# guzba/zippy

Hardware: NVIDIA H100
Metric: compress_level1_gzip_input_throughput (higher is better)
Workload: dtype u8

## Files before the change

### include/zippy_b200.h

```cpp
#ifndef ZIPPY_B200_H
#define ZIPPY_B200_H

#include <stddef.h>
#include <stdint.h>

#ifdef __cplusplus
extern "C" {
#endif

enum {
  ZB200_OK = 0,
  ZB200_ERR_INVALID_LEVEL = 1,
  ZB200_ERR_INVALID_FORMAT = 2,
  ZB200_ERR_UNCOMPRESS = 3,
  ZB200_ERR_COMPRESS = 4,
  ZB200_ERR_END_OF_BUFFER = 5,
  ZB200_ERR_BYTE_BOUNDARY = 6,
  ZB200_ERR_BLOCK_HEADER = 7,
  ZB200_ERR_INVALID_SYMBOL = 8,
  ZB200_ERR_DETECT = 9,
  ZB200_ERR_METHOD = 10,
  ZB200_ERR_CINFO = 11,
  ZB200_ERR_HEADER = 12,
  ZB200_ERR_FDICT = 13,
// ... 53 lines not shown
                                int data_format, const uint8_t *dict, size_t dict_len, uint64_t *sizes, int *statuses);
int zb200_uncompress_batch_dict(zb200_ctx *ctx, const uint8_t *src_base, const uint64_t *src_offsets, size_t n,
                                int data_format, const uint8_t *dict, size_t dict_len, uint8_t *dst_base,
                                const uint64_t *dst_offsets, uint64_t *dst_lens, int *statuses);
int zb200_decode_begin_dict(zb200_ctx *ctx, const uint8_t *src, size_t len, int data_format, const uint8_t *dict,
                            size_t dict_len, size_t *out_len);

int zb200_checksum_batch(zb200_ctx *ctx, const uint8_t *src_base, const uint64_t *src_offsets, size_t n,
                         int kind, uint32_t *out);

enum { ZB200_SYNC_FLUSH = 2, ZB200_FULL_FLUSH = 3 };
typedef struct zb200_compress_stream zb200_compress_stream;
int zb200_compress_stream_begin(zb200_ctx *ctx, int level, int data_format, int fname_len, zb200_compress_stream **out);
int zb200_compress_stream_begin_dict(zb200_ctx *ctx, int level, int data_format, const uint8_t *dict, size_t dict_len,
                                     zb200_compress_stream **out);
size_t zb200_compress_stream_bound(const zb200_compress_stream *st, size_t len);
int zb200_compress_stream_write(zb200_compress_stream *st, const uint8_t *src, size_t len,
                                uint8_t *dst, size_t dst_cap, size_t *dst_len);
int zb200_compress_stream_flush(zb200_compress_stream *st, int mode, uint8_t *dst, size_t dst_cap, size_t *dst_len);
int zb200_compress_stream_finish(zb200_compress_stream *st, uint8_t *dst, size_t dst_cap, size_t *dst_len);
void zb200_compress_stream_free(zb200_compress_stream *st);

typedef struct zb200_decompress_stream zb200_decompress_stream;
int zb200_decompress_stream_begin(zb200_ctx *ctx, int data_format, zb200_decompress_stream **out);
int zb200_decompress_stream_begin_dict(zb200_ctx *ctx, int data_format, const uint8_t *dict, size_t dict_len,
                                       zb200_decompress_stream **out);
int zb200_decompress_stream_write(zb200_decompress_stream *st, const uint8_t *src, size_t len, size_t *avail);
int zb200_decompress_stream_drain(zb200_decompress_stream *st, size_t *avail);
int zb200_decompress_stream_finish(zb200_decompress_stream *st, size_t *avail);
int zb200_decompress_stream_read(zb200_decompress_stream *st, uint8_t *dst, size_t dst_cap, size_t *dst_len);
void zb200_decompress_stream_free(zb200_decompress_stream *st);

typedef struct zb200_index zb200_index;
int zb200_index_build(zb200_ctx *ctx, const uint8_t *src, size_t len, int data_format, uint64_t span, zb200_index **out);
int zb200_index_extract_batch(zb200_ctx *ctx, const zb200_index *idx, const uint8_t *src, size_t len,
                              const uint64_t *offsets, const uint64_t *lens, size_t n, uint8_t *dst,
                              const uint64_t *dst_offsets, int *statuses);
uint64_t zb200_index_size(const zb200_index *idx);
size_t zb200_index_points(const zb200_index *idx, uint64_t *bits, uint64_t *outs, uint32_t *crcs, uint8_t *window,
                          size_t cap);
void zb200_index_free(zb200_index *idx);
int zb200_index_export(zb200_ctx *ctx, const zb200_index *idx, uint8_t *dst, size_t cap, size_t *len);
int zb200_index_import(zb200_ctx *ctx, const uint8_t *src, size_t len, zb200_index **out);

int zb200_compress_batch_device(zb200_ctx *ctx, const uint8_t *d_src, const uint64_t *src_offsets, size_t n,
                                int level, int data_format, const uint8_t *fname_lens,
                                uint8_t *d_dst, size_t dst_cap, uint64_t *dst_offsets, int *statuses);
int zb200_compress_batch_h2d(zb200_ctx *ctx, const uint8_t *src_base, const uint64_t *src_offsets, size_t n,
                             int level, int data_format, const uint8_t *fname_lens,
                             uint8_t *d_dst, size_t dst_cap, uint64_t *dst_offsets, int *statuses);
int zb200_download(zb200_ctx *ctx, const uint8_t *d_src, uint8_t *h_dst, size_t bytes);
int zb200_uncompress_batch_device(zb200_ctx *ctx, const uint8_t *d_src, const uint64_t *src_offsets, size_t n,
                                  int data_format, uint8_t *d_dst, const uint64_t *dst_offsets,
                                  uint64_t *dst_lens, int *statuses);
int zb200_uncompress_sizes_device(zb200_ctx *ctx, const uint8_t *d_src, const uint64_t *src_offsets, size_t n,
                                  int data_format, uint64_t *sizes, int *statuses);
int zb200_checksum_batch_device(zb200_ctx *ctx, const uint8_t *d_src, const uint64_t *src_offsets, size_t n,
                                int kind, uint32_t *out);

int zb200_host_register(void *ptr, size_t bytes);
int zb200_host_unregister(void *ptr);

typedef struct zb200_mgpu zb200_mgpu;
int zb200_mgpu_init(const int *devices, int n_devices, zb200_mgpu **out);
void zb200_mgpu_shutdown(zb200_mgpu *m);
int zb200_mgpu_device_count(zb200_mgpu *m);
int zb200_mgpu_compress_batch(zb200_mgpu *m, const uint8_t *src_base, const uint64_t *src_offsets, size_t n,
                              int level, int data_format, const uint8_t *fname_lens,
                              uint8_t *dst_base, size_t dst_cap, uint64_t *dst_offsets, int *statuses);
int zb200_mgpu_uncompress_batch(zb200_mgpu *m, const uint8_t *src_base, const uint64_t *src_offsets, size_t n,
                                int data_format, uint8_t *dst_base, const uint64_t *dst_offsets,
                                uint64_t *dst_lens, int *statuses);
int zb200_mgpu_checksum_batch(zb200_mgpu *m, const uint8_t *src_base, const uint64_t *src_offsets, size_t n,
                              int kind, uint32_t *out);

typedef struct {
  float lz_ms, huff_ms, scan_ms, pack_ms;
  float inflate_ms, verify_ms;
  float checksum_ms;
  float h2d_ms, d2h_ms;
  uint64_t h2d_bytes, d2h_bytes;
  uint32_t kernel_launches;
  uint32_t n_chunks;
} zb200_timing;
int zb200_last_timing(zb200_ctx *ctx, zb200_timing *out);

#ifdef __cplusplus
}
#endif
#endif
```

### zippy_b200/_native.py

```python
import ctypes
import os

_HERE = os.path.dirname(os.path.abspath(__file__))
LIB_PATH = os.path.join(_HERE, "libzippy_b200.so")

c_u8p = ctypes.c_void_p
c_u64p = ctypes.c_void_p
c_intp = ctypes.c_void_p
c_size_t = ctypes.c_size_t
c_int = ctypes.c_int


class Timing(ctypes.Structure):
    _fields_ = [("lz_ms", ctypes.c_float), ("huff_ms", ctypes.c_float), ("scan_ms", ctypes.c_float),
                ("pack_ms", ctypes.c_float), ("inflate_ms", ctypes.c_float), ("verify_ms", ctypes.c_float),
                ("checksum_ms", ctypes.c_float), ("h2d_ms", ctypes.c_float), ("d2h_ms", ctypes.c_float),
                ("h2d_bytes", ctypes.c_uint64), ("d2h_bytes", ctypes.c_uint64),
                ("kernel_launches", ctypes.c_uint32), ("n_chunks", ctypes.c_uint32)]


SYMBOLS = {
    "zb200_init": (c_int, [c_int, ctypes.POINTER(ctypes.c_void_p)]),
    "zb200_shutdown": (None, [ctypes.c_void_p]),
    "zb200_strerror": (ctypes.c_char_p, [c_int]),
    "zb200_last_cuda_error": (ctypes.c_char_p, [ctypes.c_void_p]),
    "zb200_device_count": (c_int, []),
    "zb200_set_stream": (c_int, [ctypes.c_void_p, ctypes.c_void_p]),
    "zb200_deflate_bound": (c_size_t, [c_size_t]),
    "zb200_compress_bound": (c_size_t, [c_size_t, c_int]),
    "zb200_deflate": (c_int, [ctypes.c_void_p, c_u8p, c_size_t, c_int, c_u8p, c_size_t, ctypes.POINTER(c_size_t)]),
    "zb200_inflate": (c_int, [ctypes.c_void_p, c_u8p, c_size_t, c_size_t, c_u8p, c_size_t, ctypes.POINTER(c_size_t)]),
    "zb200_inflate_size": (c_int, [ctypes.c_void_p, c_u8p, c_size_t, c_size_t, ctypes.POINTER(c_size_t)]),
    "zb200_decode_begin": (c_int, [ctypes.c_void_p, c_u8p, c_size_t, c_int, c_size_t, ctypes.POINTER(c_size_t)]),
    "zb200_decode_finish": (c_int, [ctypes.c_void_p, c_u8p, c_size_t, ctypes.POINTER(c_size_t)]),
    "zb200_crc32": (c_int, [ctypes.c_void_p, c_u8p, c_size_t, ctypes.POINTER(ctypes.c_uint32)]),
    "zb200_adler32": (c_int, [ctypes.c_void_p, c_u8p, c_size_t, ctypes.POINTER(ctypes.c_uint32)]),
    "zb200_compress_batch": (c_int, [ctypes.c_void_p, c_u8p, c_u64p, c_size_t, c_int, c_int, c_u8p, c_u8p, c_size_t,
                                     c_u64p, c_intp]),
    "zb200_compress_batch_h2d": (c_int, [ctypes.c_void_p, c_u8p, c_u64p, c_size_t, c_int, c_int, c_u8p, c_u8p, c_size_t,
                                         c_u64p, c_intp]),
    "zb200_download": (c_int, [ctypes.c_void_p, c_u8p, c_u8p, c_size_t]),
    "zb200_host_register": (c_int, [ctypes.c_void_p, c_size_t]),
    "zb200_host_unregister": (c_int, [ctypes.c_void_p]),
    "zb200_uncompress_sizes": (c_int, [ctypes.c_void_p, c_u8p, c_u64p, c_size_t, c_int, c_u64p, c_intp]),
    "zb200_uncompress_batch": (c_int, [ctypes.c_void_p, c_u8p, c_u64p, c_size_t, c_int, c_u8p, c_u64p, c_u64p, c_intp]),
    "zb200_inflate_batch_crc32": (c_int, [ctypes.c_void_p, c_u8p, c_u64p, c_size_t, c_u8p, c_u64p, c_u64p,
                                          ctypes.c_void_p, c_intp]),
    "zb200_checksum_batch": (c_int, [ctypes.c_void_p, c_u8p, c_u64p, c_size_t, c_int, ctypes.c_void_p]),
    "zb200_compress_batch_dict": (c_int, [ctypes.c_void_p, c_u8p, c_u64p, c_size_t, c_int, c_int, c_u8p, c_size_t, c_u8p,
                                          c_size_t, c_u64p, c_intp]),
    "zb200_uncompress_sizes_dict": (c_int, [ctypes.c_void_p, c_u8p, c_u64p, c_size_t, c_int, c_u8p, c_size_t, c_u64p,
                                            c_intp]),
    "zb200_uncompress_batch_dict": (c_int, [ctypes.c_void_p, c_u8p, c_u64p, c_size_t, c_int, c_u8p, c_size_t, c_u8p,
                                            c_u64p, c_u64p, c_intp]),
    "zb200_decode_begin_dict": (c_int, [ctypes.c_void_p, c_u8p, c_size_t, c_int, c_u8p, c_size_t,
                                        ctypes.POINTER(c_size_t)]),
    "zb200_compress_batch_device": (c_int, [ctypes.c_void_p, c_u8p, c_u64p, c_size_t, c_int, c_int, c_u8p, c_u8p,
                                            c_size_t, c_u64p, c_intp]),
    "zb200_uncompress_batch_device": (c_int, [ctypes.c_void_p, c_u8p, c_u64p, c_size_t, c_int, c_u8p, c_u64p, c_u64p,
                                              c_intp]),
    "zb200_uncompress_sizes_device": (c_int, [ctypes.c_void_p, c_u8p, c_u64p, c_size_t, c_int, c_u64p, c_intp]),
    "zb200_checksum_batch_device": (c_int, [ctypes.c_void_p, c_u8p, c_u64p, c_size_t, c_int, ctypes.c_void_p]),
    "zb200_compress_stream_begin": (c_int, [ctypes.c_void_p, c_int, c_int, c_int, ctypes.POINTER(ctypes.c_void_p)]),
    "zb200_compress_stream_begin_dict": (c_int, [ctypes.c_void_p, c_int, c_int, c_u8p, c_size_t,
                                                 ctypes.POINTER(ctypes.c_void_p)]),
    "zb200_compress_stream_bound": (c_size_t, [ctypes.c_void_p, c_size_t]),
    "zb200_compress_stream_write": (c_int, [ctypes.c_void_p, c_u8p, c_size_t, c_u8p, c_size_t, ctypes.POINTER(c_size_t)]),
    "zb200_compress_stream_flush": (c_int, [ctypes.c_void_p, c_int, c_u8p, c_size_t, ctypes.POINTER(c_size_t)]),
    "zb200_compress_stream_finish": (c_int, [ctypes.c_void_p, c_u8p, c_size_t, ctypes.POINTER(c_size_t)]),
    "zb200_compress_stream_free": (None, [ctypes.c_void_p]),
    "zb200_decompress_stream_begin": (c_int, [ctypes.c_void_p, c_int, ctypes.POINTER(ctypes.c_void_p)]),
    "zb200_decompress_stream_begin_dict": (c_int, [ctypes.c_void_p, c_int, c_u8p, c_size_t,
                                                   ctypes.POINTER(ctypes.c_void_p)]),
    "zb200_decompress_stream_write": (c_int, [ctypes.c_void_p, c_u8p, c_size_t, ctypes.POINTER(c_size_t)]),
    "zb200_decompress_stream_drain": (c_int, [ctypes.c_void_p, ctypes.POINTER(c_size_t)]),
    "zb200_decompress_stream_finish": (c_int, [ctypes.c_void_p, ctypes.POINTER(c_size_t)]),
    "zb200_decompress_stream_read": (c_int, [ctypes.c_void_p, c_u8p, c_size_t, ctypes.POINTER(c_size_t)]),
    "zb200_decompress_stream_free": (None, [ctypes.c_void_p]),
    "zb200_index_build": (c_int, [ctypes.c_void_p, c_u8p, c_size_t, c_int, ctypes.c_uint64,
                                  ctypes.POINTER(ctypes.c_void_p)]),
    "zb200_index_extract_batch": (c_int, [ctypes.c_void_p, ctypes.c_void_p, c_u8p, c_size_t, c_u64p, c_u64p, c_size_t,
                                          c_u8p, c_u64p, c_intp]),
    "zb200_index_size": (ctypes.c_uint64, [ctypes.c_void_p]),
    "zb200_index_points": (c_size_t, [ctypes.c_void_p, c_u64p, c_u64p, ctypes.c_void_p, c_u8p, c_size_t]),
    "zb200_index_free": (None, [ctypes.c_void_p]),
    "zb200_index_export": (c_int, [ctypes.c_void_p, ctypes.c_void_p, c_u8p, c_size_t, ctypes.POINTER(c_size_t)]),
    "zb200_index_import": (c_int, [ctypes.c_void_p, c_u8p, c_size_t, ctypes.POINTER(ctypes.c_void_p)]),
    "zb200_mgpu_init": (c_int, [ctypes.c_void_p, c_int, ctypes.POINTER(ctypes.c_void_p)]),
    "zb200_mgpu_shutdown": (None, [ctypes.c_void_p]),
    "zb200_mgpu_device_count": (c_int, [ctypes.c_void_p]),
    "zb200_mgpu_compress_batch": (c_int, [ctypes.c_void_p, c_u8p, c_u64p, c_size_t, c_int, c_int, c_u8p, c_u8p, c_size_t,
                                          c_u64p, c_intp]),
    "zb200_mgpu_uncompress_batch": (c_int, [ctypes.c_void_p, c_u8p, c_u64p, c_size_t, c_int, c_u8p, c_u64p, c_u64p, c_intp]),
    "zb200_mgpu_checksum_batch": (c_int, [ctypes.c_void_p, c_u8p, c_u64p, c_size_t, c_int, ctypes.c_void_p]),
    "zb200_last_timing": (c_int, [ctypes.c_void_p, ctypes.POINTER(Timing)]),
}

_lib = None


def lib():
# ... 14 lines not shown
```

### zippy_b200/csrc/zb_api.cu

```cuda
#include <cuda.h>
#include <cuda_runtime.h>
#include <execinfo.h>
#include <signal.h>
#include <stdio.h>
#include <unistd.h>
#include <stdlib.h>
#include <string.h>

#include <algorithm>
#include <cmath>
#include <condition_variable>
#include <deque>
#include <functional>
#include <memory>
#include <mutex>
#include <thread>
#include <string>
#include <vector>

#include "../../include/zippy_b200.h"
#include "zb_kernels.h"
#include "zb_wrapper.h"

namespace {

struct DevBuf {
  void *p = nullptr;
  size_t cap = 0;
};

struct StreamMemOps {
  CUresult (*wait32)(CUstream, CUdeviceptr, cuuint32_t, unsigned int) = nullptr;
  CUresult (*write32)(CUstream, CUdeviceptr, cuuint32_t, unsigned int) = nullptr;
  bool ok = false;
};
StreamMemOps load_stream_memops() {
  StreamMemOps m;
  void *f1 = nullptr, *f2 = nullptr;
  cudaDriverEntryPointQueryResult q1, q2;
  if (cudaGetDriverEntryPoint("cuStreamWaitValue32", &f1, cudaEnableDefault, &q1) == cudaSuccess && q1 == cudaDriverEntryPointSuccess &&
      cudaGetDriverEntryPoint("cuStreamWriteValue32", &f2, cudaEnableDefault, &q2) == cudaSuccess && q2 == cudaDriverEntryPointSuccess &&
      f1 && f2) {
    m.wait32 = reinterpret_cast<decltype(m.wait32)>(f1);
    m.write32 = reinterpret_cast<decltype(m.write32)>(f2);
    m.ok = true;
  } else {
    (void)cudaGetLastError();
  }
  return m;
}

constexpr size_t kMaxChunksPerGroup = 32768;
constexpr size_t kHostGroupChunks = 4096;
constexpr size_t ZB_STREAM_BATCH_BYTES = 64u << 20;
constexpr size_t ZB_DSTREAM_BATCH_BYTES = 64u << 20;
constexpr uint64_t kDstreamMaxOut = 1ull << 30;

}

class CopyPool {
 public:
  ~CopyPool() { stop(); }
  void start(int n) {
    if (!th_.empty()) return;
    for (int i = 0; i < n; i++) th_.emplace_back([this] { work(); });
  }
  void stop() {
    {
      std::lock_guard<std::mutex> lk(m_);
      quit_ = true;
    }
    cv_.notify_all();
    for (std::thread &t : th_) t.join();
    th_.clear();
  }
  void copy(uint8_t *dst, const uint8_t *src, size_t n) {
    const size_t piece = 1 << 20;
    if (th_.empty() || n < 2 * piece) {
      memcpy(dst, src, n);
      return;
    }
    {
      std::lock_guard<std::mutex> lk(m_);
      dst_ = dst;
      src_ = src;
      n_ = n;
      next_ = 0;
      left_ = (n + piece - 1) / piece;
    }
    cv_.notify_all();
    help(piece);
    std::unique_lock<std::mutex> lk(m_);
// ... 231 lines not shown
  return a.type == cudaMemoryTypeUnregistered;
}

int ring_ready(zb200_ctx *ctx, StageRing &r) {
  if (r.slot[0]) return ZB200_OK;
  for (int i = 0; i < kStageSlots; i++) {
    if (cudaMallocHost((void **)&r.slot[i], kStageSlotBytes) != cudaSuccess ||
        cudaEventCreateWithFlags(&r.ev[i], cudaEventDisableTiming) != cudaSuccess) {
      cudaGetLastError();
      ctx->last_err = "pinned staging ring: allocation failed";
      return ZB200_ERR_NOMEM;
    }
  }
  unsigned hc = std::thread::hardware_concurrency();
  ctx->pool.start((int)std::min<unsigned>(7, hc > 2 ? hc / 2 : 1));
  return ZB200_OK;
}

int h2d_copy(zb200_ctx *ctx, uint8_t *d_dst, const uint8_t *h_src, size_t n, cudaStream_t st, bool pageable) {
  if (!n) return ZB200_OK;
  if (!pageable) {
    CK(cudaMemcpyAsync(d_dst, h_src, n, cudaMemcpyHostToDevice, st));
    return ZB200_OK;
  }
  StageRing &r = ctx->ring_in;
  int rc = ring_ready(ctx, r);
  if (rc) return rc;
  for (size_t off = 0; off < n; off += kStageSlotBytes) {
    const size_t len = std::min(kStageSlotBytes, n - off);
    const size_t k = r.next++ % kStageSlots;
    if (r.busy[k]) CK(cudaEventSynchronize(r.ev[k]));
    ctx->pool.copy(r.slot[k], h_src + off, len);
    CK(cudaMemcpyAsync(d_dst + off, r.slot[k], len, cudaMemcpyHostToDevice, st));
    CK(cudaEventRecord(r.ev[k], st));
    r.busy[k] = true;
  }
  return ZB200_OK;
}

int d2h_complete(zb200_ctx *ctx, size_t k) {
  StageRing &r = ctx->ring_out;
  if (!r.busy[k]) return ZB200_OK;
  CK(cudaEventSynchronize(r.ev[k]));
  ctx->pool.copy(r.out_dst[k], r.slot[k], r.out_n[k]);
  r.busy[k] = false;
  return ZB200_OK;
}
int d2h_flush(zb200_ctx *ctx) {
  if (!ctx->ring_out.slot[0]) return ZB200_OK;
  for (size_t i = 0; i < (size_t)kStageSlots; i++) {
    int rc = d2h_complete(ctx, (ctx->ring_out.next + i) % kStageSlots);
    if (rc) return rc;
  }
  return ZB200_OK;
}
int d2h_copy(zb200_ctx *ctx, uint8_t *h_dst, const uint8_t *d_src, size_t n, cudaStream_t st, bool pageable) {
  if (!n) return ZB200_OK;
  if (!pageable) {
    CK(cudaMemcpyAsync(h_dst, d_src, n, cudaMemcpyDeviceToHost, st));
    return ZB200_OK;
  }
  StageRing &r = ctx->ring_out;
  int rc = ring_ready(ctx, r);
  if (rc) return rc;
  for (size_t off = 0; off < n; off += kStageSlotBytes) {
    const size_t len = std::min(kStageSlotBytes, n - off);
    const size_t k = r.next++ % kStageSlots;
    rc = d2h_complete(ctx, k);
    if (rc) return rc;
    CK(cudaMemcpyAsync(r.slot[k], d_src + off, len, cudaMemcpyDeviceToHost, st));
    CK(cudaEventRecord(r.ev[k], st));
    r.busy[k] = true;
    r.out_dst[k] = h_dst + off;
    r.out_n[k] = len;
  }
  return ZB200_OK;
}

struct Group {
  size_t m0, m1;
  size_t c0, nc;
  size_t first0;
  uint64_t in_lo, in_hi;
  uint64_t bound;
};

struct StreamPart {
  uint32_t hist;
  bool head, last;
  ZbMemberCarry carry_in, carry_out;
  bool has_dict;
  uint32_t dict_id;
};

uint32_t host_adler32(const uint8_t *p, size_t n) {
  uint64_t a = 1, b = 0;
  while (n) {
    const size_t k = std::min<size_t>(n, 5552);
    for (size_t i = 0; i < k; i++) {
      a += p[i];
      b += a;
    }
    a %= 65521;
    b %= 65521;
    p += k;
    n -= k;
  }
  return (uint32_t)(b << 16 | a);
}

struct DictScope {
  zb200_ctx *ctx;
  explicit DictScope(zb200_ctx *c) : ctx(c) {}
  int set(const uint8_t *dict, size_t dict_len, bool lz_compress = false) {
    if (!dict_len) return ZB200_OK;
    zb200_ctx *ctx = this->ctx;
    const uint32_t wl = (uint32_t)std::min<size_t>(dict_len, 32768);
    const uint8_t *w = dict + (dict_len - wl);
    if (lz_compress) {
      const uint32_t stride = zb_win16_stride(wl);
      std::vector<uint8_t> h16((size_t)16 * stride, 0);
      for (uint32_t c = 0; c < 16; c++) memcpy(h16.data() + (size_t)c * stride + ZB_WIN16_SLACK + ((c - wl) & 15u), w, wl);
      ENSURE(ctx->dict_win16, h16.size() + 64);
      CK(cudaMemcpyAsync(ctx->dict_win16.p, h16.data(), h16.size(), cudaMemcpyHostToDevice, ctx->stream));
      CK(cudaStreamSynchronize(ctx->stream));
    } else {
      ENSURE(ctx->dict_win, wl + 64);
      CK(cudaMemcpyAsync(ctx->dict_win.p, w, wl, cudaMemcpyHostToDevice, ctx->stream));
      CK(cudaStreamSynchronize(ctx->stream));
    }
    ctx->dict_len = wl;
    ctx->dict_id = host_adler32(dict, dict_len);
    ctx->dict_on = true;
    return ZB200_OK;
  }
  ~DictScope() { ctx->dict_on = false; }
};

int compress_locked(zb200_ctx *ctx, const uint8_t *d_src, const uint8_t *h_src, const uint64_t *src_offsets,
                    size_t n, int level, int data_format, const uint8_t *fname_lens, uint8_t *d_dst,
                    size_t dst_cap, uint8_t *h_dst, size_t h_dst_cap, uint64_t *dst_offsets, int *statuses,
                    size_t max_group_chunks, StreamPart *sp = nullptr) {
  if (level < -2 || level > 9) return ZB200_ERR_INVALID_LEVEL;
  if (data_format != ZB200_DF_GZIP && data_format != ZB200_DF_ZLIB && data_format != ZB200_DF_DEFLATE)
    return ZB200_ERR_INVALID_FORMAT;
  if (fname_lens)
    for (size_t i = 0; i < n; i++)
      if (fname_lens[i] > 25) return ZB200_ERR_ARG;
  if (((uintptr_t)d_dst & 3u) != 0) return ZB200_ERR_ARG;
  dst_cap &= ~(size_t)3;
  for (size_t i = 0; i < n; i++) {
    if (src_offsets[i + 1] < src_offsets[i]) return ZB200_ERR_ARG;
    if (statuses) statuses[i] = ZB200_OK;
  }
  ctx->timing.lz_ms = ctx->timing.huff_ms = ctx->timing.scan_ms = ctx->timing.pack_ms = 0.f;
  ctx->timing.n_chunks = 0;
  dst_offsets[0] = 0;
  if (n == 0) return ZB200_OK;
  const uint64_t hist = sp ? sp->hist : 0;
  const bool head = !sp || sp->head, last = !sp || sp->last;
  const bool lz = level == -1 || level >= 2;
  const bool dict_hist = !sp && ctx->dict_on && lz;
  const bool has_dict = data_format == ZB200_DF_ZLIB && (sp ? sp->has_dict : ctx->dict_on);
  const uint32_t dict_id = sp ? sp->dict_id : ctx->dict_id;
  const uint64_t src_lo = src_offsets[0] - hist;
  const bool src_pageable = h_src && is_pageable(h_src + src_lo), dst_pageable = h_dst && is_pageable(h_dst);

  std::vector<Group> groups;
  std::vector<ZbChunkDesc> desc;
  std::vector<uint32_t> first;
  size_t max_nc = 0, max_nm = 0;
  size_t chunks_left = 0;
  for (size_t i = 0; i < n; i++) {
    uint64_t len = src_offsets[i + 1] - src_offsets[i];
    chunks_left += len == 0 ? 1 : (size_t)((len + ZB_CHUNK_BYTES - 1) / ZB_CHUNK_BYTES);
  }
  const size_t group_cap = max_group_chunks;
  for (size_t m0 = 0; m0 < n;) {
    if (h_src) max_group_chunks = std::min(group_cap, std::max<size_t>(512, chunks_left / 2));
    Group g;
    g.m0 = m0;
    g.c0 = desc.size();
    g.first0 = first.size();
    g.bound = 0;
    size_t m1 = m0;
    while (m1 < n) {
      uint64_t len = src_offsets[m1 + 1] - src_offsets[m1];
      size_t nc = len == 0 ? 1 : (size_t)((len + ZB_CHUNK_BYTES - 1) / ZB_CHUNK_BYTES);
      if (desc.size() > g.c0 && desc.size() - g.c0 + nc > max_group_chunks) break;
      first.push_back((uint32_t)(desc.size() - g.c0));
      for (size_t k = 0; k < nc; k++) {
        ZbChunkDesc d;
        d.src_off = src_offsets[m1] - (h_src ? src_lo : 0) + (uint64_t)k * ZB_CHUNK_BYTES;
        d.len = (uint32_t)std::min<uint64_t>(ZB_CHUNK_BYTES, len - (uint64_t)k * ZB_CHUNK_BYTES);
        d.member = (uint32_t)(m1 - m0);
        d.flags = (k == 0 ? ZB_CHUNK_FIRST | (head ? ZB_CHUNK_HEAD : 0u) : 0u) | (k == nc - 1 && last ? ZB_CHUNK_LAST : 0u);
        d.pad = lz ? (uint32_t)std::min<uint64_t>(32768, hist + (uint64_t)k * ZB_CHUNK_BYTES) : 0u;
        if (dict_hist && k == 0) {
          d.pad = ctx->dict_len;
          d.flags |= ZB_CHUNK_DICT;
        }
        desc.push_back(d);
      }
      g.bound += zb200_compress_bound((size_t)len, data_format) + 64;
      m1++;
    }
    g.m1 = m1;
    g.nc = desc.size() - g.c0;
    chunks_left -= std::min(chunks_left, g.nc);
    first.push_back((uint32_t)g.nc);
    g.in_lo = m0 == 0 ? 0 : src_offsets[m0] - src_lo;
    g.in_hi = src_offsets[m1] - src_lo;
    max_nc = std::max(max_nc, g.nc);
    max_nm = std::max(max_nm, g.m1 - g.m0);
    groups.push_back(g);
    m0 = m1;
  }
  const size_t ng = groups.size(), nc_all = desc.size(), nfirst = first.size();

  ENSURE(ctx->desc, nc_all * sizeof(ZbChunkDesc));
  ENSURE(ctx->member_first, nfirst * sizeof(uint32_t));
  ENSURE(ctx->member_off, nfirst * sizeof(uint64_t));
  ENSURE(ctx->fname, n + 16);
  ENSURE(ctx->group_end, (ng + 1) * sizeof(uint64_t));
  ENSURE(ctx->masks, max_nc * ZB_WINDOWS_PER_CHUNK * sizeof(uint2));
  ENSURE(ctx->recs, max_nc * (size_t)ZB_RECS_PER_CHUNK * sizeof(uint32_t));
  ENSURE(ctx->hist, max_nc * (size_t)ZB_WARPS_PER_CHUNK * ZB_HIST_SYMS * sizeof(uint16_t));
  ENSURE(ctx->chk, max_nc * sizeof(ZbChunkCheck));
  ENSURE(ctx->cb, max_nc * sizeof(ZbCodebook));
  ENSURE(ctx->chunk_off, max_nc * sizeof(uint64_t));
  ENSURE(ctx->member_check, max_nm * sizeof(uint32_t));
  ENSURE(ctx->member_isize, max_nm * sizeof(uint32_t));
  if (lz) ENSURE(ctx->lz2_tables, zb_lz2_table_bytes(nullptr));
  if (sp) ENSURE(ctx->carry, 2 * sizeof(ZbMemberCarry));
  {
    int rc = ensure_pinned(ctx, nfirst * sizeof(uint64_t) + sizeof(ZbMemberCarry) + 64);
    if (rc) return rc;
    rc = ensure_group_events(ctx, 3 * ng + 1);
    if (rc) return rc;
  }
  uint64_t *pin_off = (uint64_t *)ctx->pin;
  ZbMemberCarry *pin_carry = (ZbMemberCarry *)(pin_off + nfirst);
  ZbMemberCarry *d_carry = (ZbMemberCarry *)ctx->carry.p;

  cudaStream_t s = ctx->stream;
  cudaStream_t sh = h_src ? ctx->h2d_stream : s, sd = h_dst ? ctx->d2h_stream : s;
  CK(cudaMemcpyAsync(ctx->desc.p, desc.data(), nc_all * sizeof(ZbChunkDesc), cudaMemcpyHostToDevice, s));
  CK(cudaMemcpyAsync(ctx->member_first.p, first.data(), nfirst * sizeof(uint32_t), cudaMemcpyHostToDevice, s));
  if (fname_lens && data_format == ZB200_DF_GZIP)
    CK(cudaMemcpyAsync(ctx->fname.p, fname_lens, n, cudaMemcpyHostToDevice, s));
  if (sp) CK(cudaMemcpyAsync(d_carry, &sp->carry_in, sizeof(ZbMemberCarry), cudaMemcpyHostToDevice, s));
  CK(cudaMemsetAsync(ctx->group_end.p, 0, sizeof(uint64_t), s));
  if (h_src || h_dst) {
    CK(cudaEventRecord(ctx->gev[3 * ng], s));
    if (h_src) CK(cudaStreamWaitEvent(sh, ctx->gev[3 * ng], 0));
    if (h_dst) CK(cudaStreamWaitEvent(sd, ctx->gev[3 * ng], 0));
  }
  CK(cudaEventRecord(ctx->ev[6], sh));

  auto make_work = [&](const Group &g, size_t gi) {
    ZbCompressWork w;
    w.src = d_src;
    w.dst = d_dst;
    w.dst_cap = dst_cap;
    w.desc = (const ZbChunkDesc *)ctx->desc.p + g.c0;
    w.member_first = (const uint32_t *)ctx->member_first.p + g.first0;
    w.fname_len = (fname_lens && data_format == ZB200_DF_GZIP) ? (const uint8_t *)ctx->fname.p + g.m0 : nullptr;
    w.masks = (uint2 *)ctx->masks.p;
    w.recs = (uint32_t *)ctx->recs.p;
    w.hist = (uint16_t *)ctx->hist.p;
    w.chk = (ZbChunkCheck *)ctx->chk.p;
    w.cb = (ZbCodebook *)ctx->cb.p;
    w.chunk_off = (uint64_t *)ctx->chunk_off.p;
    w.member_off = (uint64_t *)ctx->member_off.p + g.first0;
    w.member_check = (uint32_t *)ctx->member_check.p;
    w.member_isize = (uint32_t *)ctx->member_isize.p;
    w.carry_in = sp ? d_carry : nullptr;
    w.carry_out = sp ? d_carry + 1 : nullptr;
    w.tabs = ctx->d_tabs;
    w.lz2_tables = (uint2 *)ctx->lz2_tables.p;
    w.n_chunks = (uint32_t)g.nc;
    w.n_members = (uint32_t)(g.m1 - g.m0);
    w.level = level;
    w.data_format = data_format;
    w.out_base = 0;
    w.out_base_ptr = (const uint64_t *)ctx->group_end.p + gi;
    w.win16 = dict_hist ? (const uint8_t *)ctx->dict_win16.p : nullptr;
    w.win_len = dict_hist ? ctx->dict_len : 0u;
    w.win_stride = dict_hist ? zb_win16_stride(ctx->dict_len) : 0u;
    w.dict_id = dict_id;
    w.has_dict = has_dict ? 1 : 0;
    return w;
  };

  size_t d2h_done = 0;
  uint64_t total_out = 0;
  auto drain_d2h = [&](size_t upto) -> int {
    for (; d2h_done < upto; d2h_done++) {
      const Group &g = groups[d2h_done];
      CK(cudaEventSynchronize(ctx->gev[3 * d2h_done + 2]));
      const size_t nm = g.m1 - g.m0;
      const uint64_t lo = pin_off[g.first0], hi = pin_off[g.first0 + nm];
      for (size_t j = 0; j <= nm; j++) dst_offsets[g.m0 + j] = pin_off[g.first0 + j];
      total_out = hi;
      if (h_dst) {
        if (hi > h_dst_cap) return ZB200_ERR_DST_TOO_SMALL;
        CK(cudaStreamWaitEvent(sd, ctx->gev[3 * d2h_done + 1], 0));
        if (d2h_done == 0) CK(cudaEventRecord(ctx->ev[8], sd));
        if (hi > lo) {
          int rc2 = d2h_copy(ctx, h_dst + lo, d_dst + lo, (size_t)(hi - lo), sd, dst_pageable);
          if (rc2) return rc2;
        }
      }
    }
    return ZB200_OK;
  };

  for (size_t gi = 0; gi < ng; gi++) {
    const Group &g = groups[gi];
    if (h_src) {
      if (g.in_hi > g.in_lo) {
        int rc2 = h2d_copy(ctx, (uint8_t *)d_src + g.in_lo, h_src + src_lo + g.in_lo, (size_t)(g.in_hi - g.in_lo), sh, src_pageable);
        if (rc2) return rc2;
      }
      CK(cudaEventRecord(ctx->gev[3 * gi + 0], sh));
      CK(cudaStreamWaitEvent(s, ctx->gev[3 * gi + 0], 0));
    }
    ZbCompressWork w = make_work(g, gi);
    const bool timed = (gi == 0);
    if (timed) CK(cudaEventRecord(ctx->ev[0], s));
    CK(zb_launch_lz(w, s));
    if (timed) CK(cudaEventRecord(ctx->ev[1], s));
    CK(zb_launch_huff(w, s));
    if (timed) CK(cudaEventRecord(ctx->ev[2], s));
    CK(zb_launch_scan(w, s));
    if (timed) CK(cudaEventRecord(ctx->ev[3], s));
    CK(cudaMemcpyAsync((uint64_t *)ctx->group_end.p + gi + 1, w.member_off + w.n_members, sizeof(uint64_t),
                       cudaMemcpyDeviceToDevice, s));
    CK(cudaMemcpyAsync(pin_off + g.first0, w.member_off, (w.n_members + 1) * sizeof(uint64_t),
                       cudaMemcpyDeviceToHost, s));
    if (sp) CK(cudaMemcpyAsync(pin_carry, w.carry_out, sizeof(ZbMemberCarry), cudaMemcpyDeviceToHost, s));
    CK(cudaEventRecord(ctx->gev[3 * gi + 2], s));
    if (timed) CK(cudaEventRecord(ctx->ev[4], s));
    CK(zb_launch_pack(w, s));
    if (timed) CK(cudaEventRecord(ctx->ev[5], s));
    CK(cudaEventRecord(ctx->gev[3 * gi + 1], s));
    ctx->timing.kernel_launches += 5;
    ctx->timing.n_chunks += (uint32_t)g.nc;
    if (h_dst && gi >= 2) {
      int rc = drain_d2h(gi - 1);
      if (rc) return rc;
    }
  }
  if (h_src) CK(cudaEventRecord(ctx->ev[7], sh));
  {
    int rc = drain_d2h(ng);
    if (rc) return rc;
  }
  if (h_dst) CK(cudaEventRecord(ctx->ev[9], sd));
  if (dst_pageable) {
    int rc = d2h_flush(ctx);
    if (rc) return rc;
  }
  CK(cudaStreamSynchronize(s));
  if (h_src) CK(cudaStreamSynchronize(sh));
  if (h_dst) CK(cudaStreamSynchronize(sd));
  if (total_out > dst_cap) return ZB200_ERR_DST_TOO_SMALL;
  if (sp) sp->carry_out = *pin_carry;
  const float scale = groups[0].nc ? (float)nc_all / (float)groups[0].nc : 1.f;
  ctx->timing.lz_ms = ev_ms(ctx->ev[0], ctx->ev[1]) * scale;
  ctx->timing.huff_ms = ev_ms(ctx->ev[1], ctx->ev[2]) * scale;
  ctx->timing.scan_ms = ev_ms(ctx->ev[2], ctx->ev[3]) * scale;
  ctx->timing.pack_ms = ev_ms(ctx->ev[4], ctx->ev[5]) * scale;
  return ZB200_OK;
}

int stream_run(zb200_compress_stream *st, size_t nbytes, bool last, uint8_t *dst, size_t dst_cap, size_t *dst_len,
               bool reset = false) {
  zb200_ctx *ctx = st->ctx;
  if (!dst) return ZB200_ERR_DST_TOO_SMALL;
  const size_t in_end = st->hist + nbytes;
  ENSURE(ctx->in_stage, in_end + 64);
  ENSURE(ctx->out_stage, zb200_compress_bound(nbytes, st->data_format) + 128);
  const uint64_t offs[2] = {st->hist, in_end};
  uint64_t dst_offs[2] = {0, 0};
  StreamPart sp;
  sp.hist = (uint32_t)st->hist;
  sp.head = !st->head_done;
  sp.last = last;
  sp.carry_in = st->carry;
  sp.has_dict = st->has_dict;
  sp.dict_id = st->dict_id;
  int rc = compress_locked(ctx, (const uint8_t *)ctx->in_stage.p, st->buf.data(), offs, 1, st->level, st->data_format,
                           &st->fname_len, (uint8_t *)ctx->out_stage.p, ctx->out_stage.cap & ~(size_t)3, dst, dst_cap,
                           dst_offs, nullptr, ctx->host_group_chunks, &sp);
  if (rc) return rc;
  *dst_len = (size_t)dst_offs[1];
  st->carry = sp.carry_out;
  st->head_done = true;
  const bool lz = st->level == -1 || st->level >= 2;
  const size_t keep = lz && !reset ? std::min<size_t>(32768, in_end) : 0;
  st->buf.erase(st->buf.begin(), st->buf.begin() + (in_end - keep));
  st->hist = keep;
  return ZB200_OK;
}

int upload_pieces(zb200_ctx *ctx, const uint64_t *offs, size_t n, ZbChecksumWork &w) {
  std::vector<ZbPiece> pieces;
  std::vector<uint32_t> first(n + 1);
  for (size_t i = 0; i < n; i++) {
    first[i] = (uint32_t)pieces.size();
    uint64_t cap = offs[i + 1] - offs[i];
    uint64_t rel = 0;
// ... 3080 lines not shown
```

### zippy_b200/csrc/zb_deflate.cu

```cuda
#include "zb_device.cuh"
#include "zb_kernels.h"
#include "zb_huff_warp.cuh"

#define LZ_THREADS (ZB_WARPS_PER_CHUNK * 32)
#define LZ_HASH_BITS 11
#define LZ_TABLE_ENTRIES (1 << LZ_HASH_BITS)
#define LZ_PRESEED 2048
#ifndef ZB_LZ1_RESOLVE_WINNER
#define ZB_LZ1_RESOLVE_WINNER 0
#endif
#define LZ_LANE_CAP 32

#define LZ_PIECE_BYTES ZB_REC_PIECE_BYTES
#define LZ_PHASES (ZB_SUB_BYTES / LZ_PIECE_BYTES)
#define LZ_PHASE_BYTES (ZB_CHUNK_BYTES / LZ_PHASES)
#define LZ_PHASE_HIST 1024
#define LZ_BATCH_LPW 2
#define LZ_BATCH_WINDOWS (32 / LZ_BATCH_LPW)
static_assert(LZ_PIECE_BYTES * ZB_WARPS_PER_CHUNK == LZ_PHASE_BYTES, "one piece per warp and phase");
static_assert(LZ_PIECE_BYTES / ZB_WINDOW % LZ_BATCH_WINDOWS == 0, "a batch of windows never straddles two pieces");

#define LZ_SM_DATA 0
#define LZ_SM_DATA_BYTES (LZ_PHASE_BYTES + LZ_PHASE_HIST + 64 + 384)
#define LZ_SM_TABLE (LZ_SM_DATA + LZ_SM_DATA_BYTES)
// ... 967 lines not shown
    } else if (w.data_format == ZB_DF_ZLIB) {
      t[0] = (uint8_t)(ck >> 24); t[1] = (uint8_t)(ck >> 16); t[2] = (uint8_t)(ck >> 8); t[3] = (uint8_t)ck;
    }
  }

  if (btype == 0) {
    uint8_t *o = w.dst + out0;
    uint32_t npieces = len == 0 ? 1u : (len + 65534u) / 65535u;
    for (uint32_t pc = 0; pc < npieces; pc++) {
      uint32_t s0 = pc * 65535u, n = min(65535u, len - s0);
      uint8_t *ob = o + (size_t)pc * 5u + s0;
      if (tid == 0) {
        ob[0] = (uint8_t)((cb->is_final && pc == npieces - 1) ? 1 : 0);
        ob[1] = (uint8_t)n; ob[2] = (uint8_t)(n >> 8);
        ob[3] = (uint8_t)~n; ob[4] = (uint8_t)((~n) >> 8);
      }
      for (uint32_t i = (uint32_t)tid; i < n; i += LZ_THREADS) ob[5 + i] = src[s0 + i];
    }
    return;
  }

  const uint64_t gbit0 = out0 * 8ull;
  const uint32_t B0 = (uint32_t)(gbit0 & 31ull);
  uint32_t *dstw_rel = reinterpret_cast<uint32_t *>(w.dst) + (gbit0 >> 5);
  const uint32_t end_bit = B0 + cb->total_bytes * 8u;
  if (tid < PK_EDGES) {
    uint32_t b = tid == 0 ? B0 : tid <= 7 ? B0 + cb->warp_bit_start[tid] : tid == 8 ? B0 + cb->eob_bit_start : end_bit;
    ed.word[tid] = b >> 5;
    ed.val[tid] = 0u;
    ed.used[tid] = 0u;
  }
  __syncthreads();

  const uint32_t piece_start = warp == 0 ? B0 : B0 + cb->warp_bit_start[warp];
  {
    uint32_t *rows = rows_all + warp * PK_ROW_WORDS * 32;
    uint32_t *stg = stg_all + warp * PK_STG_WORDS;
    uint32_t bitcur = piece_start, sw0 = piece_start >> 5;
    if (warp == 0) {
      const uint32_t hb = cb->hdr_bits;
      for (uint32_t base = 0; base < hb; base += 1024u) {
        const uint32_t k = (base >> 5) + (uint32_t)lane;
        uint32_t piece = 0, nb = 0;
        if (k * 32u < hb) {
          for (int j = 0; j < 4; j++) piece |= (uint32_t)cb->hdr[k * 4 + j] << (8 * j);
          nb = min(32u, hb - k * 32u);
        }
        rows[lane] = piece;
        __syncwarp();
        pk_append(stg, rows, nb, bitcur, sw0, piece_start, dstw_rel, &ed);
      }
    }
    const uint32_t b0 = (uint32_t)warp * ZB_SUB_BYTES;
    if (b0 < len) {
      const uint32_t b1 = min(b0 + ZB_SUB_BYTES, len);
      const uint2 *gmask = w.masks + (size_t)chunk * ZB_WINDOWS_PER_CHUNK;
      const uint32_t *grecs = w.recs + (size_t)chunk * ZB_RECS_PER_CHUNK + (size_t)warp * ZB_RECS_PER_SUB;
      const uint32_t nwin = (b1 - b0 + 31u) >> 5;
      const uint32_t mis = (uint32_t)(uintptr_t)(src + b0) & 3u;
      uint32_t rec_base = 0;
      for (uint32_t wbase = 0; wbase < nwin; wbase += 32) {
        if (wbase && (wbase & (ZB_REC_PIECE_WINDOWS - 1u)) == 0u) {
          grecs += ZB_REC_PIECE_BYTES / 4;
          rec_base = 0;
        }
        const uint32_t widx = wbase + (uint32_t)lane;
        const uint32_t win = (b0 >> 5) + widx;
        uint2 mk = make_uint2(0u, 0u);
        if (widx < nwin) mk = gmask[win];
        uint32_t s = mk.x;
        const uint32_t im = mk.y;
        const uint32_t nmatch = (uint32_t)__popc(im);
        uint32_t rincl = nmatch;
#pragma unroll
        for (int o = 1; o < 32; o <<= 1) {
          const uint32_t t = __shfl_up_sync(ZB_FULL, rincl, o);
          if (lane >= o) rincl += t;
        }
        const uint32_t rtot = __shfl_sync(ZB_FULL, rincl, 31);
        {
          const uint32_t bbase = b0 + (wbase << 5);
          const uint32_t *pw = reinterpret_cast<const uint32_t *>(src + bbase - mis);
          const uint32_t nword = min(1024u, b1 - bbase) + mis;
#pragma unroll 1
          for (uint32_t k = (uint32_t)lane; 4u * k < nword; k += 32) {
            const uint32_t v = __ldg(pw + k);
            uint32_t *q = stg + PK_LIT_OFF + k + (k >> 3);
            if (k < 256u) *q = v;
            if (k && (k & 7u) == 0u) q[-1] = v;
          }
          const uint32_t *brec = grecs + rec_base;
#pragma unroll 1
          for (uint32_t k = (uint32_t)lane; k < rtot; k += 32) stg[PK_REC_OFF + k] = brec[k];
        }
        rec_base += rtot;
        __syncwarp();
        const uint8_t *lit = reinterpret_cast<const uint8_t *>(stg + PK_LIT_OFF + lane * PK_SLOT_WORDS) + mis;
        uint32_t ri = PK_REC_OFF + rincl - nmatch;
        uint32_t wi = (uint32_t)lane, acc = 0, accn = 0;
        while (s) {
          const uint32_t t1 = s & (0u - s);
          s ^= t1;
          const uint32_t t2 = s & (0u - s);
          const uint32_t l1 = lit[31 - __clz(t1)], l2 = lit[31 - __clz(t2)];
          const uint32_t r = stg[ri];
          const bool is_m = (im & t1) != 0u;
          const bool pair = t2 != 0u && (im & (t1 | t2)) == 0u;
          s ^= pair ? t2 : 0u;
          ri += is_m ? 1u : 0u;
          const uint32_t rec = is_m ? r : 0u;
          const uint32_t sym1 = is_m ? 257u + (rec & 31u) : l1;
          const uint32_t sym2 = is_m ? 288u + ((rec >> 10) & 31u) : pair ? l2 : PK_CODE_NONE;
          const uint32_t e1 = codes[sym1], e2 = codes[sym2];
          pk_put(rows, (e1 & 0xffffu) | ((rec >> 5) & 31u) << __byte_perm(e1, 0u, 0x4442), e1 >> 24, acc, accn, wi);
          pk_put(rows, (e2 & 0xffffu) | (rec >> 15) << __byte_perm(e2, 0u, 0x4442), e2 >> 24, acc, accn, wi);
        }
        rows[wi] = acc;
        __syncwarp();
        for (uint32_t k = (uint32_t)lane; k < PK_REC_OFF - PK_LIT_OFF + rtot; k += 32) stg[PK_LIT_OFF + k] = 0u;
        __syncwarp();
        pk_append(stg, rows, wi - (uint32_t)lane + accn, bitcur, sw0, piece_start, dstw_rel, &ed);
      }
    }
    if (lane == 0 && (bitcur & 31u)) pk_edge_or(&ed, sw0, stg[0]);
  }
  if (tid == 96) {
    const uint32_t e = codes[256];
    uint32_t pos = B0 + cb->eob_bit_start;
    unsigned long long tv = (unsigned long long)(e & 0xffffu);
    uint32_t nb = e >> 24;
    if (!cb->is_final) {
      nb += 3u;
      nb += (8u - ((pos + nb) & 7u)) & 7u;
      tv |= 0xffff0000ull << nb;
      nb += 32u;
    } else {
      nb += (8u - ((pos + nb) & 7u)) & 7u;
    }
    while (nb) {
      const uint32_t rel = pos >> 5, sh = pos & 31u, take = min(nb, 32u - sh);
      const uint32_t bits = (uint32_t)(tv & ((1ull << take) - 1ull)) << sh;
      if (sh == 0 && take == 32u) dstw_rel[rel] = bits;
      else pk_edge_or(&ed, rel, bits);
      tv >>= take;
      pos += take;
      nb -= take;
    }
  }
  __syncthreads();
  if (tid < PK_EDGES && ed.used[tid] && (tid == 0 || ed.word[tid] != ed.word[tid - 1])) {
    const uint32_t rel = ed.word[tid], val = ed.val[tid];
    const uint32_t lo = rel * 32u, hi = lo + 32u;
    if (lo >= B0 && hi <= end_bit) dstw_rel[rel] = val;
    else {
      uint8_t *bp = reinterpret_cast<uint8_t *>(dstw_rel + rel);
      for (uint32_t j = 0; j < 4; j++)
        if (lo + 8u * j >= B0 && lo + 8u * j + 8u <= end_bit) bp[j] = (uint8_t)(val >> (8u * j));
    }
  }
}

static bool zb_is_lz_level(int level) { return level == -1 || level >= 2; }
ZbLz2Params zb_lz2_params(int level) {
  static const ZbLz2Params table[10] = {{4, 4, 4, 8, 16}, {4, 4, 4, 8, 16}, {2, 4, 2, 4, 0},  {2, 4, 3, 4, 6},   {3, 4, 3, 4, 8},
                                        {3, 4, 4, 8, 16}, {4, 4, 4, 8, 16}, {4, 4, 6, 8, 32}, {4, 4, 8, 16, 32}, {4, 4, 8, 32, 64}};
  return table[(level >= 2 && level <= 9) ? level : 6];
}
size_t zb_lz2_table_bytes(int *grid_out) {
  int grid = LZ2_CTAS_PER_SM * zb_sm_count();
  if (grid_out) *grid_out = grid;
  return (size_t)grid * LZ2_TABLES_PER_CTA * LZ2_BUCKETS * sizeof(uint2);
}
typedef void (*ZbLzKernel)(const uint8_t *, const ZbChunkDesc *, uint2 *, uint32_t *, uint16_t *, ZbChunkCheck *,
                           const ZbCrcTables *);
static ZbLzKernel zb_lz_kernel(int mode, int data_format) {
  const int ck = data_format == ZB_DF_GZIP ? ZB_CK_CRC : data_format == ZB_DF_ZLIB ? ZB_CK_ADLER : 0;
// ... 55 lines not shown
```

Before: 77.56.

## Plan chunks into pinned memory and batch literal staging loads in pack kernel

```diff
diff --git a/include/zippy_b200.h b/include/zippy_b200.h
--- a/include/zippy_b200.h
+++ b/include/zippy_b200.h
@@ -159,6 +159,7 @@
   uint64_t h2d_bytes, d2h_bytes;
   uint32_t kernel_launches;
   uint32_t n_chunks;
+  float plan_ms;
 } zb200_timing;
 int zb200_last_timing(zb200_ctx *ctx, zb200_timing *out);
 
diff --git a/zippy_b200/_native.py b/zippy_b200/_native.py
--- a/zippy_b200/_native.py
+++ b/zippy_b200/_native.py
@@ -16,7 +16,7 @@
                 ("pack_ms", ctypes.c_float), ("inflate_ms", ctypes.c_float), ("verify_ms", ctypes.c_float),
                 ("checksum_ms", ctypes.c_float), ("h2d_ms", ctypes.c_float), ("d2h_ms", ctypes.c_float),
                 ("h2d_bytes", ctypes.c_uint64), ("d2h_bytes", ctypes.c_uint64),
-                ("kernel_launches", ctypes.c_uint32), ("n_chunks", ctypes.c_uint32)]
+                ("kernel_launches", ctypes.c_uint32), ("n_chunks", ctypes.c_uint32), ("plan_ms", ctypes.c_float)]
 
 
 SYMBOLS = {
diff --git a/zippy_b200/csrc/zb_api.cu b/zippy_b200/csrc/zb_api.cu
--- a/zippy_b200/csrc/zb_api.cu
+++ b/zippy_b200/csrc/zb_api.cu
@@ -8,6 +8,7 @@
 #include <string.h>
 
 #include <algorithm>
+#include <chrono>
 #include <cmath>
 #include <condition_variable>
 #include <deque>
@@ -405,7 +406,6 @@
   size_t c0, nc;
   size_t first0;
   uint64_t in_lo, in_hi;
-  uint64_t bound;
 };
 
 struct StreamPart {
@@ -464,6 +464,7 @@
                     size_t n, int level, int data_format, const uint8_t *fname_lens, uint8_t *d_dst,
                     size_t dst_cap, uint8_t *h_dst, size_t h_dst_cap, uint64_t *dst_offsets, int *statuses,
                     size_t max_group_chunks, StreamPart *sp = nullptr) {
+  const auto t_entry = std::chrono::steady_clock::now();
   if (level < -2 || level > 9) return ZB200_ERR_INVALID_LEVEL;
   if (data_format != ZB200_DF_GZIP && data_format != ZB200_DF_ZLIB && data_format != ZB200_DF_DEFLATE)
     return ZB200_ERR_INVALID_FORMAT;
@@ -472,11 +473,8 @@
       if (fname_lens[i] > 25) return ZB200_ERR_ARG;
   if (((uintptr_t)d_dst & 3u) != 0) return ZB200_ERR_ARG;
   dst_cap &= ~(size_t)3;
-  for (size_t i = 0; i < n; i++) {
-    if (src_offsets[i + 1] < src_offsets[i]) return ZB200_ERR_ARG;
-    if (statuses) statuses[i] = ZB200_OK;
-  }
-  ctx->timing.lz_ms = ctx->timing.huff_ms = ctx->timing.scan_ms = ctx->timing.pack_ms = 0.f;
+  if (src_offsets[n] < src_offsets[0]) return ZB200_ERR_ARG;
+  ctx->timing.lz_ms = ctx->timing.huff_ms = ctx->timing.scan_ms = ctx->timing.pack_ms = ctx->timing.plan_ms = 0.f;
   ctx->timing.n_chunks = 0;
   dst_offsets[0] = 0;
   if (n == 0) return ZB200_OK;
@@ -489,31 +487,41 @@
   const uint64_t src_lo = src_offsets[0] - hist;
   const bool src_pageable = h_src && is_pageable(h_src + src_lo), dst_pageable = h_dst && is_pageable(h_dst);
 
+  auto chunks_of = [](uint64_t len) { return len == 0 ? (size_t)1 : (size_t)((len + ZB_CHUNK_BYTES - 1) / ZB_CHUNK_BYTES); };
+  const size_t nc_cap = n + (size_t)((src_offsets[n] - src_offsets[0]) / ZB_CHUNK_BYTES), nfirst_cap = 2 * n;
+  {
+    int rc = ensure_pinned(ctx, nfirst_cap * (sizeof(uint64_t) + sizeof(uint32_t)) + sizeof(ZbMemberCarry) +
+                                    nc_cap * sizeof(ZbChunkDesc) + 64);
+    if (rc) return rc;
+  }
+  uint64_t *pin_off = (uint64_t *)ctx->pin;
+  ZbMemberCarry *pin_carry = (ZbMemberCarry *)(pin_off + nfirst_cap);
+  ZbChunkDesc *desc = (ZbChunkDesc *)(pin_carry + 1);
+  uint32_t *first = (uint32_t *)(desc + nc_cap);
   std::vector<Group> groups;
-  std::vector<ZbChunkDesc> desc;
-  std::vector<uint32_t> first;
   size_t max_nc = 0, max_nm = 0;
+  size_t nd = 0, nfirst = 0;
   size_t chunks_left = 0;
-  for (size_t i = 0; i < n; i++) {
-    uint64_t len = src_offsets[i + 1] - src_offsets[i];
-    chunks_left += len == 0 ? 1 : (size_t)((len + ZB_CHUNK_BYTES - 1) / ZB_CHUNK_BYTES);
-  }
+  if (h_src)
+    for (size_t i = 0; i < n; i++) chunks_left += chunks_of(src_offsets[i + 1] - src_offsets[i]);
   const size_t group_cap = max_group_chunks;
   for (size_t m0 = 0; m0 < n;) {
     if (h_src) max_group_chunks = std::min(group_cap, std::max<size_t>(512, chunks_left / 2));
     Group g;
     g.m0 = m0;
-    g.c0 = desc.size();
-    g.first0 = first.size();
-    g.bound = 0;
+    g.c0 = nd;
+    g.first0 = nfirst;
     size_t m1 = m0;
     while (m1 < n) {
+      if (src_offsets[m1 + 1] < src_offsets[m1]) return ZB200_ERR_ARG;
       uint64_t len = src_offsets[m1 + 1] - src_offsets[m1];
-      size_t nc = len == 0 ? 1 : (size_t)((len + ZB_CHUNK_BYTES - 1) / ZB_CHUNK_BYTES);
-      if (desc.size() > g.c0 && desc.size() - g.c0 + nc > max_group_chunks) break;
-      first.push_back((uint32_t)(desc.size() - g.c0));
+      size_t nc = chunks_of(len);
+      if (nd + nc > nc_cap) return ZB200_ERR_ARG;
+      if (nd > g.c0 && nd - g.c0 + nc > max_group_chunks) break;
+      if (statuses) statuses[m1] = ZB200_OK;
+      first[nfirst++] = (uint32_t)(nd - g.c0);
       for (size_t k = 0; k < nc; k++) {
-        ZbChunkDesc d;
+        ZbChunkDesc &d = desc[nd++];
         d.src_off = src_offsets[m1] - (h_src ? src_lo : 0) + (uint64_t)k * ZB_CHUNK_BYTES;
         d.len = (uint32_t)std::min<uint64_t>(ZB_CHUNK_BYTES, len - (uint64_t)k * ZB_CHUNK_BYTES);
         d.member = (uint32_t)(m1 - m0);
@@ -523,15 +531,13 @@
           d.pad = ctx->dict_len;
           d.flags |= ZB_CHUNK_DICT;
         }
-        desc.push_back(d);
       }
-      g.bound += zb200_compress_bound((size_t)len, data_format) + 64;
       m1++;
     }
     g.m1 = m1;
-    g.nc = desc.size() - g.c0;
+    g.nc = nd - g.c0;
     chunks_left -= std::min(chunks_left, g.nc);
-    first.push_back((uint32_t)g.nc);
+    first[nfirst++] = (uint32_t)g.nc;
     g.in_lo = m0 == 0 ? 0 : src_offsets[m0] - src_lo;
     g.in_hi = src_offsets[m1] - src_lo;
     max_nc = std::max(max_nc, g.nc);
@@ -539,7 +545,7 @@
     groups.push_back(g);
     m0 = m1;
   }
-  const size_t ng = groups.size(), nc_all = desc.size(), nfirst = first.size();
+  const size_t ng = groups.size(), nc_all = nd;
 
   ENSURE(ctx->desc, nc_all * sizeof(ZbChunkDesc));
   ENSURE(ctx->member_first, nfirst * sizeof(uint32_t));
@@ -557,19 +563,19 @@
   if (lz) ENSURE(ctx->lz2_tables, zb_lz2_table_bytes(nullptr));
   if (sp) ENSURE(ctx->carry, 2 * sizeof(ZbMemberCarry));
   {
-    int rc = ensure_pinned(ctx, nfirst * sizeof(uint64_t) + sizeof(ZbMemberCarry) + 64);
+    int rc = ensure_group_events(ctx, 3 * ng + 1);
     if (rc) return rc;
-    rc = ensure_group_events(ctx, 3 * ng + 1);
-    if (rc) return rc;
-  }
-  uint64_t *pin_off = (uint64_t *)ctx->pin;
-  ZbMemberCarry *pin_carry = (ZbMemberCarry *)(pin_off + nfirst);
+  }
   ZbMemberCarry *d_carry = (ZbMemberCarry *)ctx->carry.p;
 
   cudaStream_t s = ctx->stream;
   cudaStream_t sh = h_src ? ctx->h2d_stream : s, sd = h_dst ? ctx->d2h_stream : s;
-  CK(cudaMemcpyAsync(ctx->desc.p, desc.data(), nc_all * sizeof(ZbChunkDesc), cudaMemcpyHostToDevice, s));
-  CK(cudaMemcpyAsync(ctx->member_first.p, first.data(), nfirst * sizeof(uint32_t), cudaMemcpyHostToDevice, s));
+  struct SyncOnReturn {
+    cudaStream_t s;
+    ~SyncOnReturn() { cudaStreamSynchronize(s); }
+  } sync_on_return{s};
+  CK(cudaMemcpyAsync(ctx->desc.p, desc, nc_all * sizeof(ZbChunkDesc), cudaMemcpyHostToDevice, s));
+  CK(cudaMemcpyAsync(ctx->member_first.p, first, nfirst * sizeof(uint32_t), cudaMemcpyHostToDevice, s));
   if (fname_lens && data_format == ZB200_DF_GZIP)
     CK(cudaMemcpyAsync(ctx->fname.p, fname_lens, n, cudaMemcpyHostToDevice, s));
   if (sp) CK(cudaMemcpyAsync(d_carry, &sp->carry_in, sizeof(ZbMemberCarry), cudaMemcpyHostToDevice, s));
@@ -651,7 +657,10 @@
     }
     ZbCompressWork w = make_work(g, gi);
     const bool timed = (gi == 0);
-    if (timed) CK(cudaEventRecord(ctx->ev[0], s));
+    if (timed) {
+      ctx->timing.plan_ms = std::chrono::duration<float, std::milli>(std::chrono::steady_clock::now() - t_entry).count();
+      CK(cudaEventRecord(ctx->ev[0], s));
+    }
     CK(zb_launch_lz(w, s));
     if (timed) CK(cudaEventRecord(ctx->ev[1], s));
     CK(zb_launch_huff(w, s));
diff --git a/zippy_b200/csrc/zb_deflate.cu b/zippy_b200/csrc/zb_deflate.cu
--- a/zippy_b200/csrc/zb_deflate.cu
+++ b/zippy_b200/csrc/zb_deflate.cu
@@ -1073,16 +1073,23 @@
           const uint32_t bbase = b0 + (wbase << 5);
           const uint32_t *pw = reinterpret_cast<const uint32_t *>(src + bbase - mis);
           const uint32_t nword = min(1024u, b1 - bbase) + mis;
-#pragma unroll 1
-          for (uint32_t k = (uint32_t)lane; 4u * k < nword; k += 32) {
-            const uint32_t v = __ldg(pw + k);
+          uint32_t v[8];
+#pragma unroll
+          for (uint32_t j = 0; j < 8; j++) {
+            const uint32_t k = (uint32_t)lane + 32u * j;
+            v[j] = 4u * k < nword ? __ldg(pw + k) : 0u;
+          }
+#pragma unroll
+          for (uint32_t j = 0; j < 8; j++) {
+            const uint32_t k = (uint32_t)lane + 32u * j;
             uint32_t *q = stg + PK_LIT_OFF + k + (k >> 3);
-            if (k < 256u) *q = v;
-            if (k && (k & 7u) == 0u) q[-1] = v;
+            if (4u * k < nword) *q = v[j];
+            if (4u * k < nword && k && (k & 7u) == 0u) q[-1] = v[j];
           }
+          if (lane == 0 && 4u * 256u < nword) stg[PK_LIT_OFF + 256 + 32 - 1] = __ldg(pw + 256);
           const uint32_t *brec = grecs + rec_base;
-#pragma unroll 1
-          for (uint32_t k = (uint32_t)lane; k < rtot; k += 32) stg[PK_REC_OFF + k] = brec[k];
+#pragma unroll 4
+          for (uint32_t k = (uint32_t)lane; k < rtot; k += 32) stg[PK_REC_OFF + k] = __ldg(brec + k);
         }
         rec_base += rtot;
         __syncwarp();
```

New measurement: 80.81 (median of 6 runs). +4.2%, better.
